# evgueni-ovtchinnikov/raleigh

Hardware: AMD Instinct MI355X
Metric: inner-iter GB/s vs HBM roofline (Gram+dots+SpMM of one block-JCG iteration) (higher is better)
Workload: dtype f64; 1 GPU; block-JCG inner iteration: 9 Gram + 4 dots + 1 SpMM, n=215x215x215=9938375 rows (9938375 per GPU), m=32, 7-pt Laplacian nnz=69291275, rows sharded over 1 GPU(s), strong scaling; n=9938375, m=32, nnz=69291275

## Files before the change

### raleigh_amd/csrc/gram.hip

```cpp
#include <stdlib.h>

#include "common.h"

namespace rlh {

template <typename R> struct Mfma16;
template <> struct Mfma16<double> {
  typedef double acc_t __attribute__((ext_vector_type(4)));
  static __device__ __forceinline__ acc_t run(double a, double b, acc_t c) {
    return __builtin_amdgcn_mfma_f64_16x16x4f64(a, b, c, 0, 0, 0);
  }
  static __device__ __forceinline__ int out_row(int lane, int reg) { return (lane >> 4) + 4 * reg; }
};
template <> struct Mfma16<float> {
  typedef float acc_t __attribute__((ext_vector_type(4)));
  static __device__ __forceinline__ acc_t run(float a, float b, acc_t c) {
    return __builtin_amdgcn_mfma_f32_16x16x4f32(a, b, c, 0, 0, 0);
  }
  static __device__ __forceinline__ int out_row(int lane, int reg) { return (lane >> 4) * 4 + reg; }
};

struct GramSeg { const void *p; int64_t ld; int c0; };
constexpr int kGramSegs = 4;

// ... 889 lines not shown
    a.npj = (vx + 127) / 128;
    a.nchunks = (n + 256 / (int)sizeof(R) - 1) / (256 / (int)sizeof(R));
    if (a.same && vx <= 128)
      return gram_launch<DT, 4, 2, true, 0, false, true, true>(a, 1, 1, my, mx, d_out);
    return gram_launch<DT, 4, 2, true, 0, false, true>(a, (vy + 127) / 128, a.npj, my, mx, d_out);
  }
  if (aligned && vx > 32 && vy > 32 && vx <= 64 && vy <= 64 && env_quad()) {
    a.npj = 1;
    a.nchunks = (n + 512 / (int)sizeof(R) - 1) / (512 / (int)sizeof(R));
    if (a.same) return gram_launch<DT, 2, 1, true, 0, false, true, true>(a, 1, 1, my, mx, d_out);
    return gram_launch<DT, 2, 1, true, 0, false, true>(a, 1, 1, my, mx, d_out);
  }
  const int ROWS = (mode == 3 ? 2 : (mode == 4 ? 4 : 1)) * 512 / (int)sizeof(R);
  a.nchunks = (n + ROWS - 1) / ROWS;
#define RLH_GRAM_CASE(pi, pj)                                                              \
  if (PI == pi && PJ == pj) {                                                              \
    if constexpr (pi * pj <= 4)        \
      if (mode == 1) return gram_launch<DT, pi, pj, true, 1>(a, npi, npj, my, mx, d_out);  \
    if constexpr (pi <= 2 && pj <= 2)         \
      if (mode == 3) return gram_launch<DT, pi, pj, true, 3>(a, npi, npj, my, mx, d_out);  \
    if constexpr (pi * pj == 1)                                                            \
      if (mode == 4) return gram_launch<DT, pi, pj, true, 4>(a, npi, npj, my, mx, d_out);  \
    if constexpr (pi == pj && pi <= 2)                                                     \
      if (mode == 2) return gram_launch<DT, pi, pj, true, 2>(a, npi, npj, my, mx, d_out);  \
    return aligned ? gram_launch<DT, pi, pj, true, 0>(a, npi, npj, my, mx, d_out)          \
                   : gram_launch<DT, pi, pj, false, 0>(a, npi, npj, my, mx, d_out);        \
  }
  RLH_GRAM_CASE(1, 1) RLH_GRAM_CASE(1, 2) RLH_GRAM_CASE(1, 4)
  RLH_GRAM_CASE(2, 1) RLH_GRAM_CASE(2, 2) RLH_GRAM_CASE(2, 4)
  RLH_GRAM_CASE(4, 1) RLH_GRAM_CASE(4, 2) RLH_GRAM_CASE(4, 4)
#undef RLH_GRAM_CASE
  set_error("rlh_gram: no kernel for panel %d x %d", PI, PJ);
  return 1;
}

template <int DT>
static int gram_multi_impl(int64_t n, int nx, const void *const *X, const int64_t *ldx, const int64_t *mx, int ny,
                           const void *const *Y, const int64_t *ldy, const int64_t *my, void *d_out) {
  using R = typename DType<DT>::R;
  constexpr int NC = DType<DT>::cplx ? 2 : 1;
  Context &c = ctx();
  GramArgs a;
  const int64_t es = dtype_size(DT);
  bool aligned = true;
  int64_t mxt = 0, myt = 0;
  for (int k = 0; k < nx; ++k) {
    a.xs[k] = GramSeg{X[k], ldx[k], (int)mxt};
    mxt += mx[k];
    aligned = aligned && aligned16(X[k], ldx[k], es);
  }
  for (int k = 0; k < ny; ++k) {
    a.ys[k] = GramSeg{Y[k], ldy[k], (int)myt};
    myt += my[k];
    aligned = aligned && aligned16(Y[k], ldy[k], es);
  }
  for (int k = nx; k < kGramSegs; ++k) a.xs[k] = GramSeg{nullptr, 0, 1 << 30};
  for (int k = ny; k < kGramSegs; ++k) a.ys[k] = GramSeg{nullptr, 0, 1 << 30};
  a.nxs = nx; a.nys = ny;
  const int vx = (int)mxt * NC, vy = (int)myt * NC;
  const int PI = pick_tiles(vy), PJ = pick_tiles(vx);
  const int npi = (vy + PI * 16 - 1) / (PI * 16), npj = (vx + PJ * 16 - 1) / (PJ * 16);
  a.X = X[0]; a.Y = Y[0]; a.ldx = ldx[0]; a.ldy = ldy[0]; a.n = n; a.mx = (int)mxt; a.my = (int)myt;
  a.same = 0; a.npj = npj; a.partials = c.work;
  a.nt = gram_nt(n * (mxt + myt) * es);
  {
    const int stream = getenv("RLH_GRAM_STREAM") ? atoi(getenv("RLH_GRAM_STREAM")) : 1;
    if (stream && aligned && vx <= 64 && vy <= 64 && (vx > 8 || vy > 8)) {
      a.npj = 1;
      a.xal = -1;
      if (!DType<DT>::cplx && nx == 1 && mxt > 16 && mxt <= 32 && myt > 32)
        for (int k2 = 0; k2 < ny; ++k2)
          if (Y[k2] == X[0] && ldy[k2] == ldx[0] && my[k2] == mx[0] && a.ys[k2].c0 % 16 == 0) a.xal = a.ys[k2].c0;
      return gram_stream_launch<DT>(a, myt, mxt, d_out);
    }
  }
  if (nx == 1 && npi * npj > 1) {
    for (int k = 0; k < ny; ++k)
      if (int rc = gram_impl<DT>(n, mx[0], X[0], ldx[0], my[k], Y[k], ldy[k],
                                 (char *)d_out + (size_t)a.ys[k].c0 * (size_t)mxt * (size_t)es))
        return rc;
    return 0;
  }
  const int ROWS = 512 / (int)sizeof(R);
  a.nchunks = (n + ROWS - 1) / ROWS;
#define RLH_GRAM_MCASE(pi, pj)                                                                        \
  if (PI == pi && PJ == pj)                                                                           \
    return aligned ? gram_launch<DT, pi, pj, true, 0, true>(a, npi, npj, myt, mxt, d_out)             \
                   : gram_launch<DT, pi, pj, false, 0, true>(a, npi, npj, myt, mxt, d_out);
  RLH_GRAM_MCASE(1, 1) RLH_GRAM_MCASE(1, 2) RLH_GRAM_MCASE(1, 4)
  RLH_GRAM_MCASE(2, 1) RLH_GRAM_MCASE(2, 2) RLH_GRAM_MCASE(2, 4)
  RLH_GRAM_MCASE(4, 1) RLH_GRAM_MCASE(4, 2) RLH_GRAM_MCASE(4, 4)
#undef RLH_GRAM_MCASE
  set_error("rlh_gram_multi: no kernel for panel %d x %d", PI, PJ);
  return 1;
}

template <typename T, bool ALIGNED, bool NT>
__global__ __launch_bounds__(256) void dots_kernel(const T *X, int64_t ldx, const T *Y, int64_t ldy, int64_t n,
                                                   T *partials, int nbx, int per) {
  constexpr int VEC = 16 / (int)sizeof(T);
  const int col = blockIdx.y;
  const T *x = X + (int64_t)col * ldx;
  const T *y = Y + (int64_t)col * ldy;
  T acc = zero_of(T{});
  struct alignas(16) V { T v[VEC]; };
  typedef unsigned u4 __attribute__((ext_vector_type(4)));
  auto piece = [&](const T *p) -> V {
    union { u4 u; V v; } c;
    if constexpr (NT) c.u = __builtin_nontemporal_load(reinterpret_cast<const u4 *>(p));
    else c.u = *reinterpret_cast<const u4 *>(p);
    return c.v;
  };
  for (int g = 0; g < per; g += 4) {
    const int64_t base = ((int64_t)blockIdx.x * per + g) * 256 * VEC;
    if (base >= n) break;
    if (ALIGNED && base + 4 * 256 * VEC <= n && x == y) {
      V xv[4];
#pragma unroll
      for (int i = 0; i < 4; ++i) xv[i] = piece(x + base + ((int64_t)i * 256 + threadIdx.x) * VEC);
#pragma unroll
      for (int i = 0; i < 4; ++i)
#pragma unroll
        for (int e = 0; e < VEC; ++e) fma_conj_acc(acc, xv[i].v[e], xv[i].v[e]);
    } else if (ALIGNED && base + 4 * 256 * VEC <= n) {
      V xv[4], yv[4];
#pragma unroll
      for (int i = 0; i < 4; ++i) {
        const int64_t r = base + ((int64_t)i * 256 + threadIdx.x) * VEC;
        xv[i] = piece(x + r);
        yv[i] = piece(y + r);
      }
#pragma unroll
      for (int i = 0; i < 4; ++i)
#pragma unroll
        for (int e = 0; e < VEC; ++e) fma_conj_acc(acc, yv[i].v[e], xv[i].v[e]);
    } else {
      for (int i = 0; i < 4; ++i) {
        const int64_t r = base + ((int64_t)i * 256 + threadIdx.x) * VEC;
        for (int e = 0; e < VEC && r + e < n; ++e) fma_conj_acc(acc, y[r + e], x[r + e]);
      }
    }
  }
  __shared__ T red[256];
  red[threadIdx.x] = acc;
  __syncthreads();
  for (int s = 128; s > 0; s >>= 1) {
    if (threadIdx.x < s) red[threadIdx.x] = add_of(red[threadIdx.x], red[threadIdx.x + s]);
    __syncthreads();
  }
  if (threadIdx.x == 0) partials[(int64_t)col * nbx + blockIdx.x] = red[0];
}

template <typename T>
__global__ __launch_bounds__(256) void dots_finalize(const T *partials, int nbx, int m, T *out) {
  const int lane = threadIdx.x & 63;
  const int col = blockIdx.x * 4 + (threadIdx.x >> 6);
  if (col >= m) return;
  T s = zero_of(T{});
  for (int b = lane; b < nbx; b += 64) s = add_of(s, partials[(int64_t)col * nbx + b]);
  if constexpr (sizeof(T) == sizeof(float) || sizeof(T) == sizeof(double)) {
    using R = T;
#pragma unroll
    for (int off = 32; off > 0; off >>= 1) s = s + (R)__shfl_xor(s, off);
  }
  if (lane == 0) out[col] = s;
}

template <typename R2, typename C>
__device__ __forceinline__ C shfl_complex(C v, int off) {
  C r;
  r.re = __shfl_xor(v.re, off);
  r.im = __shfl_xor(v.im, off);
  return r;
}

template <>
__global__ __launch_bounds__(256) void dots_finalize<c32>(const c32 *partials, int nbx, int m, c32 *out) {
  const int lane = threadIdx.x & 63;
  const int col = blockIdx.x * 4 + (threadIdx.x >> 6);
  if (col >= m) return;
  c32 s = zero_of(c32{});
  for (int b = lane; b < nbx; b += 64) s = add_of(s, partials[(int64_t)col * nbx + b]);
#pragma unroll
  for (int off = 32; off > 0; off >>= 1) s = add_of(s, shfl_complex<float>(s, off));
  if (lane == 0) out[col] = s;
}

template <>
__global__ __launch_bounds__(256) void dots_finalize<c64>(const c64 *partials, int nbx, int m, c64 *out) {
  const int lane = threadIdx.x & 63;
  const int col = blockIdx.x * 4 + (threadIdx.x >> 6);
  if (col >= m) return;
  c64 s = zero_of(c64{});
  for (int b = lane; b < nbx; b += 64) s = add_of(s, partials[(int64_t)col * nbx + b]);
#pragma unroll
  for (int off = 32; off > 0; off >>= 1) s = add_of(s, shfl_complex<double>(s, off));
  if (lane == 0) out[col] = s;
}

template <int DT>
static int dots_impl(int64_t n, int64_t m, const void *X, int64_t ldx, const void *Y, int64_t ldy, void *d_out) {
  using T = typename DType<DT>::T;
  Context &c = ctx();
  constexpr int VEC = 16 / (int)sizeof(T);
  int per = 4;
  int64_t nbx = (n + 256 * VEC * (int64_t)per - 1) / (256 * VEC * (int64_t)per);
  while (nbx > 2048 || (nbx > 1 && (size_t)nbx * m * sizeof(T) > kWorkspaceBytes / 4)) {
    per += 4;
    nbx = (n + 256 * VEC * (int64_t)per - 1) / (256 * VEC * (int64_t)per);
  }
  if (nbx < 1) nbx = 1;
  RLH_REQUIRE((size_t)nbx * m * sizeof(T) <= kWorkspaceBytes, "rlh_dots: too many columns");
  const int nt = gram_nt(n * m * (int64_t)sizeof(T) * (X == Y ? 1 : 2));
  const bool aligned = aligned16(X, ldx, sizeof(T)) && aligned16(Y, ldy, sizeof(T));
  dim3 grid((unsigned)nbx, (unsigned)m);
  if (aligned && (nt & 1))
    hipLaunchKernelGGL((dots_kernel<T, true, true>), grid, dim3(256), 0, c.stream, (const T *)X, ldx, (const T *)Y, ldy,
                       n, (T *)c.work, (int)nbx, per);
  else if (aligned)
    hipLaunchKernelGGL((dots_kernel<T, true, false>), grid, dim3(256), 0, c.stream, (const T *)X, ldx, (const T *)Y, ldy,
                       n, (T *)c.work, (int)nbx, per);
  else
    hipLaunchKernelGGL((dots_kernel<T, false, false>), grid, dim3(256), 0, c.stream, (const T *)X, ldx, (const T *)Y, ldy,
                       n, (T *)c.work, (int)nbx, per);
  RLH_HIP(hipGetLastError());
  hipLaunchKernelGGL((dots_finalize<T>), dim3(((int)m + 3) / 4), dim3(256), 0, c.stream, (const T *)c.work,
                     (int)nbx, (int)m, (T *)d_out);
  RLH_HIP(hipGetLastError());
  return 0;
}

template <typename R>
__global__ __launch_bounds__(256) void absmax_kernel(const R *X, int64_t ldx_r, int64_t n_r, double *partials, int nbx) {
  const R *x = X + (int64_t)blockIdx.y * ldx_r;
  double mx = 0.0;
  const int64_t stride = (int64_t)gridDim.x * 256;
  for (int64_t r = (int64_t)blockIdx.x * 256 + threadIdx.x; r < n_r; r += stride) {
    const double v = fabs((double)x[r]);
    mx = v > mx ? v : mx;
  }
  __shared__ double red[256];
  red[threadIdx.x] = mx;
  __syncthreads();
  for (int s = 128; s > 0; s >>= 1) {
    if (threadIdx.x < s) red[threadIdx.x] = red[threadIdx.x] > red[threadIdx.x + s] ? red[threadIdx.x] : red[threadIdx.x + s];
    __syncthreads();
  }
  if (threadIdx.x == 0) partials[(int64_t)blockIdx.y * nbx + blockIdx.x] = red[0];
}

__global__ __launch_bounds__(256) void absmax_finalize(const double *partials, int64_t count, double *out) {
  double mx = 0.0;
  for (int64_t i = threadIdx.x; i < count; i += 256) mx = partials[i] > mx ? partials[i] : mx;
  __shared__ double red[256];
  red[threadIdx.x] = mx;
  __syncthreads();
  for (int s = 128; s > 0; s >>= 1) {
    if (threadIdx.x < s) red[threadIdx.x] = red[threadIdx.x] > red[threadIdx.x + s] ? red[threadIdx.x] : red[threadIdx.x + s];
    __syncthreads();
  }
  if (threadIdx.x == 0) out[0] = red[0];
}

template <int DT>
static int absmax_impl(int64_t n, int64_t m, const void *X, int64_t ldx, void *d_out) {
  using R = typename DType<DT>::R;
  constexpr int NC = DType<DT>::cplx ? 2 : 1;
  Context &c = ctx();
  int64_t nbx = (n * NC + 256 * 8 - 1) / (256 * 8);
  const int64_t cap = ((int64_t)c.num_cu * 8 + m - 1) / m;
  if (nbx > cap) nbx = cap;
  if (nbx < 1) nbx = 1;
  RLH_REQUIRE((size_t)nbx * m * sizeof(double) <= kWorkspaceBytes, "rlh_absmax: too many columns");
  hipLaunchKernelGGL((absmax_kernel<R>), dim3((unsigned)nbx, (unsigned)m), dim3(256), 0, c.stream, (const R *)X,
                     ldx * NC, n * NC, (double *)c.work, (int)nbx);
  RLH_HIP(hipGetLastError());
  hipLaunchKernelGGL(absmax_finalize, dim3(1), dim3(256), 0, c.stream, (const double *)c.work, nbx * m, (double *)d_out);
  RLH_HIP(hipGetLastError());
  return 0;
}

template <typename T>
__global__ __launch_bounds__(256) void dots_transp_kernel(const T *X, int64_t ldx, const T *Y, int64_t ldy,
                                                          int64_t n, int m, T *out) {
  const int64_t stride = (int64_t)gridDim.x * blockDim.x;
  for (int64_t r = (int64_t)blockIdx.x * blockDim.x + threadIdx.x; r < n; r += stride) {
    T acc = zero_of(T{});
    for (int i = 0; i < m; ++i) fma_conj_acc(acc, Y[r + (int64_t)i * ldy], X[r + (int64_t)i * ldx]);
    out[r] = acc;
  }
}

template <int DT>
static int dots_transp_impl(int64_t n, int64_t m, const void *X, int64_t ldx, const void *Y, int64_t ldy,
                            void *d_out) {
  using T = typename DType<DT>::T;
  Context &c = ctx();
  int64_t nb = (n + 255) / 256;
  if (nb > (int64_t)c.num_cu * 8) nb = (int64_t)c.num_cu * 8;
  hipLaunchKernelGGL((dots_transp_kernel<T>), dim3((unsigned)nb), dim3(256), 0, c.stream, (const T *)X, ldx,
                     (const T *)Y, ldy, n, (int)m, (T *)d_out);
  RLH_HIP(hipGetLastError());
  return 0;
}

}

using namespace rlh;

#define RLH_DISPATCH(dt, fn, ...)                              \
  switch (dt) {                                                \
    case RLH_S: rc = fn<RLH_S>(__VA_ARGS__); break;            \
    case RLH_D: rc = fn<RLH_D>(__VA_ARGS__); break;            \
    case RLH_C: rc = fn<RLH_C>(__VA_ARGS__); break;            \
    case RLH_Z: rc = fn<RLH_Z>(__VA_ARGS__); break;            \
    default: rlh::set_error("unknown dtype %d", dt); rc = 1;   \
  }

extern "C" {

int rlh_gram(int dtype, int64_t n, int64_t mx, const void *X, int64_t ldx, int64_t my, const void *Y, int64_t ldy,
             void *d_out, void *h_out) {
  if (int rc = require_ready()) return rc;
  RLH_REQUIRE(dtype_valid(dtype), "rlh_gram: unknown dtype %d", dtype);
  RLH_REQUIRE(n >= 0 && mx >= 0 && my >= 0, "rlh_gram: negative size");
  RLH_REQUIRE(mx <= 32768 && my <= 32768, "rlh_gram: more than 32768 vectors in a window");
  if (mx == 0 || my == 0) return 0;
  RLH_REQUIRE(X && Y, "rlh_gram: null block pointer");
  RLH_REQUIRE(ldx >= n && ldy >= n, "rlh_gram: leading dimension smaller than n");
  RLH_REQUIRE(d_out || h_out, "rlh_gram: no output buffer");
  const size_t bytes = (size_t)(mx * my * dtype_size(dtype));
  if (!d_out) {
    if (int rc = ensure_result(bytes)) return rc;
    d_out = ctx().result_hd;
  }
  int rc = 0;
  if (n == 0) {
    RLH_HIP(hipMemsetAsync(d_out, 0, bytes, ctx().stream));
  } else {
    RLH_DISPATCH(dtype, gram_impl, n, mx, X, ldx, my, Y, ldy, d_out)
  }
  if (rc) return rc;
  if (h_out) return fetch_result(h_out, d_out, bytes);
  return 0;
}

int rlh_gram_multi(int dtype, int64_t n, int nx, const void *const *X, const int64_t *ldx, const int64_t *mx, int ny,
// ... 89 lines not shown
```

### raleigh_amd/csrc/spmm.hip

```cpp
#include <unordered_map>

#include "spmm.h"

namespace rlh {

template <typename T, int JT, int TT, bool CHEB>
__global__ __launch_bounds__(256, (JT * TT >= 64 ? 1 : 2)) void sell_spmm_kernel(const int64_t *__restrict__ slice_ptr,
                                                        const int32_t *__restrict__ cols,
                                                        const T *__restrict__ vals, int64_t n_rows,
                                                        int64_t n_slices, const T *__restrict__ X, int64_t ldx,
                                                        int64_t n_own, const T *__restrict__ H, int64_t ldh,
                                                        T *__restrict__ Y, int64_t ldy, int m, int chunk,
                                                        int ntiles, int tiles_per_block, ChebArgs<T> cheb) {
  const int lane = threadIdx.x & 63;
  const int wave = threadIdx.x >> 6;
  const int xcd = blockIdx.x & 7;
  const int slices_per_block = 4 / tiles_per_block;
  const int64_t q0 = (int64_t)(blockIdx.x >> 3) * slices_per_block + wave / tiles_per_block;
  const int64_t q_stride = (int64_t)(gridDim.x >> 3) * slices_per_block;
  const int64_t nchunks = (n_slices + chunk - 1) / chunk;
  for (int tile = wave % tiles_per_block; tile < ntiles; tile += tiles_per_block) {
    const int j0 = tile * JT;
    const int jv = (m - j0) < JT ? (m - j0) : JT;
    const T *__restrict__ Xp = X + (int64_t)j0 * ldx;
// ... 443 lines not shown
      scol[i] = gsrc[mt.goff + g + lane / LPG] + (lane % LPG) * EPL;
    }
    auto stage_load = [&](int s, VecU<T, EPL> (&st)[SLOTS]) {
#pragma unroll
      for (int i = 0; i < SLOTS; ++i) {
        int j = s * cps + scc[i];
        if (j > m - 1) j = m - 1;
        st[i] = *reinterpret_cast<const VecU<T, EPL> *>(X + (int64_t)j * ldx + scol[i]);
      }
    };
    auto stage_write = [&](int s, const VecU<T, EPL> (&st)[SLOTS]) {
      unsigned boff = (unsigned)(s & 1) * (unsigned)kStkBufBytes;
      asm volatile("" : "+s"(boff));
#pragma unroll
      for (int i = 0; i < SLOTS; ++i) {
        VecA<T, EPL> val;
#pragma unroll
        for (int k = 0; k < EPL; ++k) val.e[k] = st[i].e[k];
        *reinterpret_cast<VecA<T, EPL> *>(ldsb + (lane16 + (boff + (unsigned)sbase[i]))) = val;
      }
    };
    auto compute = [&](int s) {
      unsigned boff = (unsigned)(s & 1) * (unsigned)kStkBufBytes;
      int j = s * cps;
      const int jend = (j + cps < m) ? j + cps : m;
      for (; j < jend; ++j) {
        asm volatile("" : "+s"(boff));
#pragma unroll
        for (int r = 0; r < R; ++r) {
          T acc = zero_of(T{});
#pragma unroll
          for (int t = 0; t < WMAX; ++t) {
            if constexpr (!PACK) {
              fma_acc(acc, v[r][t], *reinterpret_cast<const T *>(ldsb + (ixb[r][t] + boff)));
            } else if ((t & 1) == 0) {
              unsigned w = ixb[r][t / 2];
              asm volatile("" : "+v"(w));
              fma_acc(acc, v[r][t], *reinterpret_cast<const T *>(ldsb + ((w & 0xffffu) * (unsigned)sizeof(T) + boff)));
              fma_acc(acc, v[r][t + 1], *reinterpret_cast<const T *>(ldsb + ((w >> 16) * (unsigned)sizeof(T) + boff)));
            }
          }
          if (row[r] < n_rows) nt_store(Y + row[r] + (int64_t)j * ldy, acc);
        }
        boff += (unsigned)F * (unsigned)sizeof(T);
      }
    };
    if constexpr (sizeof(T) >= 8) {
      VecU<T, EPL> stA[SLOTS];
      stage_load(0, stA);
      stage_write(0, stA);
      __syncthreads();
      for (int s = 0; s + 1 < nsteps; ++s) {
        stage_load(s + 1, stA);
        compute(s);
        stage_write(s + 1, stA);
        __syncthreads();
      }
      compute(nsteps - 1);
      __syncthreads();
      continue;
    }
    VecU<T, EPL> stA[SLOTS], stB[SLOTS];
    stage_load(0, stA);
    stage_load(nsteps > 1 ? 1 : 0, stB);
    stage_write(0, stA);
    __syncthreads();
    int s = 0;
    for (; s + 3 < nsteps; s += 2) {
      stage_load(s + 2, stA);
      compute(s);
      stage_write(s + 1, stB);
      __syncthreads();
      stage_load(s + 3, stB);
      compute(s + 1);
      stage_write(s + 2, stA);
      __syncthreads();
    }
    const int left = nsteps - s;
    if (left == 3) {
      stage_load(s + 2, stA);
      compute(s);
      stage_write(s + 1, stB);
      __syncthreads();
      compute(s + 1);
      stage_write(s + 2, stA);
      __syncthreads();
      compute(s + 2);
    } else if (left == 2) {
      compute(s);
      stage_write(s + 1, stB);
      __syncthreads();
      compute(s + 1);
    } else {
      compute(s);
    }
    __syncthreads();
  }
}

template <int N> __device__ __forceinline__ void wait_vm_le() { asm volatile("s_waitcnt vmcnt(%0)" :: "n"(N) : "memory"); }

__device__ __forceinline__ void wait_vm_outstanding(int n) {
#define RLH_WC(k) case k: wait_vm_le<k>(); break;
#define RLH_WC8(k) RLH_WC(k) RLH_WC(k + 1) RLH_WC(k + 2) RLH_WC(k + 3) RLH_WC(k + 4) RLH_WC(k + 5) RLH_WC(k + 6) RLH_WC(k + 7)
  switch (n) {
    RLH_WC8(0) RLH_WC8(8) RLH_WC8(16)
    default: wait_vm_le<0>(); break;
  }
#undef RLH_WC8
#undef RLH_WC
}

constexpr int kStkLdsBytes = 160 * 1024;
template <typename T> struct StkRing { static constexpr int NB = sizeof(T) >= 16 ? 2 : 4, SLOT = kStkLdsBytes / NB; };

__device__ __forceinline__ void stk_touch(float &v) { asm volatile("" : "+v"(v)); }
__device__ __forceinline__ void stk_touch(double &v) { asm volatile("" : "+v"(v)); }
__device__ __forceinline__ void stk_touch(c32 &v) { asm volatile("" : "+v"(v.re), "+v"(v.im)); }
__device__ __forceinline__ void stk_touch(c64 &v) { asm volatile("" : "+v"(v.re), "+v"(v.im)); }

__device__ __forceinline__ void stk_store(float *p, float v) { __builtin_nontemporal_store(v, p); }
__device__ __forceinline__ void stk_store(double *p, double v) { __builtin_nontemporal_store(v, p); }
__device__ __forceinline__ void stk_store(c32 *p, c32 v) {
  typedef float f32x2 __attribute__((ext_vector_type(2)));
  __builtin_nontemporal_store(f32x2{v.re, v.im}, reinterpret_cast<f32x2 *>(p));
}
__device__ __forceinline__ void stk_store(c64 *p, c64 v) {
  typedef double f64x2 __attribute__((ext_vector_type(2)));
  __builtin_nontemporal_store(f64x2{v.re, v.im}, reinterpret_cast<f64x2 *>(p));
}

template <typename T, int R, int LD, int DBG = 0, bool CHEB = false>
__global__ __launch_bounds__(1024) void well_stack_dma_kernel(const WellMeta *__restrict__ meta,
                                                              const int32_t *__restrict__ member,
                                                              const int32_t *__restrict__ gsrc,
                                                              const uint16_t *__restrict__ idx,
                                                              const T *__restrict__ vals, const int32_t *__restrict__ pat,
                                                              const uint16_t *__restrict__ dtab, int64_t n_rows,
                                                              const int32_t *__restrict__ sched, int64_t sched_len,
                                                              const T *__restrict__ X, int64_t ldx, int64_t n_own,
                                                              const T *__restrict__ H, int64_t ldh,
                                                              T *__restrict__ Y, int64_t ldy, int m, ChebArgs<T> cheb) {
  constexpr int WMAX = 8;
  constexpr int NB = StkRing<T>::NB, D = NB - 1;
  static_assert(!CHEB || NB == 2, "the fused step drains the ring every vector: two slots only");
  constexpr int SLOT = StkRing<T>::SLOT;
  constexpr int EPL = 16 / (int)sizeof(T);
  constexpr int LPG = 64 / EPL;
  static_assert((D - 1) * LD + D * R < 24, "wait_vm_outstanding's cases");
  extern __shared__ __align__(16) char ldsb[];
  const int tid = threadIdx.x;
  const int lane = tid & 63;
  const int wave = __builtin_amdgcn_readfirstlane(tid >> 6);
  for (int64_t pos = blockIdx.x; pos < sched_len; pos += gridDim.x) {
    const int64_t sb = sched[pos];
    if (sb < 0) continue;
    const WellMeta mt = meta[sb];
    const int ng = mt.width_ng >> 8;
    int row[R];
    T v[R][WMAX];
    unsigned ixb[R][WMAX / 2];
    bool whole = true;
    int nmem = 0;
#pragma unroll
    for (int r = 0; r < R; ++r) {
      const int2 mr = reinterpret_cast<const int2 *>(member)[sb * R + r];
      if (mr.y > 0) {
        nmem = r + 1;
        whole = whole && mr.y == kWellRows;
      }
      row[r] = tid < mr.y ? mr.x + tid : -1;
      unsigned px[WMAX];
      if (sizeof(T) < 16 && pat) well_load_entries_pat<T, WMAX>(vals, pat, dtab, idx, mt.eoff + 8 * r, sb * R + r, tid, v[r], px);
      else well_load_entries<T, WMAX>(vals, idx, mt.eoff + 8 * r, tid, WMAX, v[r], px);
#pragma unroll
      for (int t = 0; t < WMAX; t += 2) ixb[r][t / 2] = px[t] | (px[t + 1] << 16);
    }
    int scol[LD];
    const int npieces = ng / EPL;
    const int nw = __builtin_amdgcn_readfirstlane((npieces + LD - 1) / LD);
    const int mine = __builtin_amdgcn_readfirstlane(wave < nw ? (npieces - wave + nw - 1) / nw : 0);
#pragma unroll
    for (int i = 0; i < LD; ++i) {
      int q = (wave + nw * i) * EPL;
      if (q > ng - EPL) q = ng - EPL;
      scol[i] = gsrc[mt.goff + q + lane / LPG] + (lane % LPG) * EPL;
    }
#pragma unroll
    for (int r = 0; r < R; ++r) {
#pragma unroll
      for (int t = 0; t < WMAX; ++t) stk_touch(v[r][t]);
#pragma unroll
      for (int t = 0; t < WMAX / 2; ++t) asm volatile("" : "+v"(ixb[r][t]));
    }
#pragma unroll
    for (int i = 0; i < LD; ++i) asm volatile("" : "+v"(scol[i]));
    auto issue = [&](int j) {
      const unsigned slot = (unsigned)(j & (NB - 1)) * (unsigned)SLOT;
      const T *src = X + (int64_t)j * ldx;
      const T *hsrc = H ? H + (int64_t)j * ldh - n_own : src;
#pragma unroll
      for (int i = 0; i < LD; ++i) {
        if (i >= mine || (DBG & 1)) break;
        const T *g = (scol[i] < n_own ? src : hsrc) + scol[i];
        unsigned dst = slot + (unsigned)(wave + nw * i) * 1024u, keep;
        asm volatile("s_mov_b32 %0, m0\n\ts_mov_b32 m0, %2\n\ts_nop 0\n\tglobal_load_lds_dwordx4 %1, off\n\ts_mov_b32 m0, %0"
                     : "=&s"(keep) : "v"(g), "s"(dst) : "memory");
      }
    };
    auto compute = [&](int j) {
      unsigned boff = (unsigned)(j & (NB - 1)) * (unsigned)SLOT;
      asm volatile("" : "+s"(boff));
#pragma unroll
      for (int r = 0; r < R; ++r) {
        if (r >= nmem) break;
        T acc = zero_of(T{});
#pragma unroll
        for (int t = 0; t < WMAX; t += 2) {
          unsigned w = ixb[r][t / 2];
          asm volatile("" : "+v"(w));
          if constexpr ((DBG & 2) != 0) acc = (t == (j & 6)) ? v[r][t] : acc;
          else {
            fma_acc(acc, v[r][t], *reinterpret_cast<const T *>(ldsb + ((w & 0xffffu) * (unsigned)sizeof(T) + boff)));
            fma_acc(acc, v[r][t + 1], *reinterpret_cast<const T *>(ldsb + ((w >> 16) * (unsigned)sizeof(T) + boff)));
          }
        }
        if constexpr ((DBG & 4) != 0) { if (ixb[r][0] == 0xfffffffeu) Y[(int64_t)row[r] + (int64_t)j * ldy] = acc; }
        else if constexpr ((DBG & 8) != 0) { if (whole || row[r] >= 0) Y[(int64_t)row[r] + (int64_t)j * ldy] = acc; }
        else if (whole || row[r] >= 0) stk_store(Y + (int64_t)row[r] + (int64_t)j * ldy, acc);
      }
    };
    __builtin_amdgcn_s_barrier();
    if constexpr (CHEB) {
      issue(0);
      for (int j = 0; j < m; ++j) {
        if (j == 0) wait_vm_outstanding(0);
        __builtin_amdgcn_s_barrier();
        if (j + 1 < m) issue(j + 1);
        unsigned boff = (unsigned)(j & (NB - 1)) * (unsigned)SLOT;
        asm volatile("" : "+s"(boff));
#pragma unroll
        for (int r = 0; r < R; ++r) {
          if (r >= nmem) break;
          T acc = zero_of(T{});
#pragma unroll
          for (int t = 0; t < WMAX - 2; t += 2) {
            unsigned w = ixb[r][t / 2];
            asm volatile("" : "+v"(w));
            fma_acc(acc, v[r][t], *reinterpret_cast<const T *>(ldsb + ((w & 0xffffu) * (unsigned)sizeof(T) + boff)));
            fma_acc(acc, v[r][t + 1], *reinterpret_cast<const T *>(ldsb + ((w >> 16) * (unsigned)sizeof(T) + boff)));
          }
          unsigned w = ixb[r][WMAX / 2 - 1];
          asm volatile("" : "+v"(w));
          fma_acc(acc, v[r][WMAX - 2], *reinterpret_cast<const T *>(ldsb + ((w & 0xffffu) * (unsigned)sizeof(T) + boff)));
          const T yv = *reinterpret_cast<const T *>(ldsb + ((w >> 16) * (unsigned)sizeof(T) + boff));
          T out = sub_of(scale_of(cheb.cy, yv), scale_of(cheb.cb, acc));
          const bool live = whole || row[r] >= 0;
          T *pp = Y + (int64_t)row[r] + (int64_t)j * ldy;
          T pv = zero_of(T{}), bv = zero_of(T{});
          if (live) {
            pv = *pp;
            bv = cheb.B[(int64_t)row[r] + (int64_t)j * cheb.ldb];
          }
          wait_vm_outstanding(0);
          stk_touch(pv);
          stk_touch(bv);
          out = add_of(add_of(out, scale_of(cheb.cp, pv)), scale_of(cheb.cb, bv));
          if (live) stk_store(pp, out);
        }
      }
      continue;
    }
    for (int j = 0; j < D && j < m; ++j) issue(j);
    for (int j = 0; j < m; ++j) {
      const int later = m - 1 - j < D - 1 ? m - 1 - j : D - 1;
      wait_vm_outstanding(((DBG & 1) ? 0 : later * mine) + ((DBG & 16) && whole ? (j < D ? j : D) * nmem : 0));
      __builtin_amdgcn_s_barrier();
      if (j + D < m) issue(j + D);
      compute(j);
    }
  }
}

__device__ __forceinline__ float bf16_to_f32(unsigned short h) { return __uint_as_float((unsigned)h << 16); }
__device__ __forceinline__ unsigned short f32_to_bf16(float f) {
  unsigned u = __float_as_uint(f);
  u += 0x7FFFu + ((u >> 16) & 1u);
  return (unsigned short)(u >> 16);
}
__device__ __forceinline__ float cheb_update(float cy, float y, float cp, float p, float cb, float b, float t) {
  return __fmaf_rn(cy, y, __fmaf_rn(cp, p, __fmul_rn(cb, __fsub_rn(b, t))));
}
struct alignas(16) Bf8 { unsigned short e[8]; };
struct alignas(8) Bf8U { unsigned short e[8]; };

constexpr int kBfCps = 8;
constexpr int kBfBufBytes = 56 * 1024;

template <int WMAX>
__global__ __launch_bounds__(1024) void well_cheb_bf16_kernel(const WellMeta *__restrict__ meta,
                                                              const int32_t *__restrict__ gsrc,
                                                              const uint16_t *__restrict__ idx,
                                                              const float *__restrict__ vals, int64_t n_rows,
                                                              const int32_t *__restrict__ sched, int64_t sched_len,
                                                              const unsigned short *__restrict__ Yk, int64_t ldy,
                                                              int64_t n_own, const unsigned short *__restrict__ H,
                                                              int64_t ldh,
                                                              unsigned short *__restrict__ P, int64_t ldp,
                                                              const unsigned short *__restrict__ B, int64_t ldb,
                                                              int m, float cy, float cp, float cb) {
  constexpr int SLOTS = 4;
  __shared__ __attribute__((aligned(16))) char ldsb[2 * kBfBufBytes + 16 * kBfCps * 64 * 4];
  const int tid = threadIdx.x;
  const int lane = tid & 63;
  const int wave = __builtin_amdgcn_readfirstlane(tid >> 6);
  float *tile = reinterpret_cast<float *>(ldsb + 2 * kBfBufBytes) + wave * (kBfCps * 64);
  for (int64_t pos = blockIdx.x; pos < sched_len; pos += gridDim.x) {
    const int64_t b = sched[pos];
    if (b < 0) continue;
    const WellMeta mt = meta[b];
    const int width = mt.width_ng & 255;
    const int ng = mt.width_ng >> 8;
    const int F2 = ng * 128;
    int cps = kBfBufBytes / F2;
    if (cps > kBfCps) cps = kBfCps;
    if (cps > m) cps = m;
    const int nsteps = (m + cps - 1) / cps;
    const int G = ng * cps;
    const int64_t row0 = b * kWellRows + (int64_t)wave * 64;
    const int64_t row = row0 + lane;
    float v[WMAX];
    unsigned ixb[WMAX];
    well_load_entries<float, WMAX>(vals, idx, mt.eoff, tid, width, v, ixb);
#pragma unroll
    for (int t = 0; t < WMAX; ++t) ixb[t] *= 2u;
    int sbase[SLOTS], scc[SLOTS], scol[SLOTS];
#pragma unroll
    for (int i = 0; i < SLOTS; ++i) {
      int q = (wave + 16 * i) * 8;
      if (q > G - 8) q = G - 8;
      const int cc = q / ng, g = q - cc * ng;
      scc[i] = __builtin_amdgcn_readfirstlane(cc);
      sbase[i] = __builtin_amdgcn_readfirstlane(cc * F2 + g * 128);
      scol[i] = gsrc[mt.goff + g + lane / 8] + (lane % 8) * 8;
    }
    Bf8U stA[SLOTS], stB[SLOTS];
    auto stage_load = [&](int s, Bf8U (&st)[SLOTS]) {
#pragma unroll
      for (int i = 0; i < SLOTS; ++i) {
        int j = s * cps + scc[i];
        if (j > m - 1) j = m - 1;
        const int c = scol[i];
        const unsigned short *src = c < n_own ? Yk + (int64_t)j * ldy + c : H + (int64_t)j * ldh + (c - n_own);
        st[i] = *reinterpret_cast<const Bf8U *>(src);
      }
    };
    auto stage_write = [&](int s, const Bf8U (&st)[SLOTS]) {
      unsigned boff = (unsigned)(s & 1) * (unsigned)kBfBufBytes;
      asm volatile("" : "+s"(boff));
#pragma unroll
      for (int i = 0; i < SLOTS; ++i) {
        Bf8 val;
#pragma unroll
        for (int k = 0; k < 8; ++k) val.e[k] = st[i].e[k];
        *reinterpret_cast<Bf8 *>(ldsb + ((unsigned)lane * 16u + (boff + (unsigned)sbase[i]))) = val;
      }
    };
    auto compute = [&](int s) {
      unsigned boff = (unsigned)(s & 1) * (unsigned)kBfBufBytes;
      const int j0 = s * cps;
      const int c8 = lane >> 3, rg = lane & 7;
      const int j = j0 + c8;
      const int64_t r8 = row0 + rg * 8;
      const bool mine = c8 < cps && j < m && r8 < n_rows;
      const bool whole = mine && r8 + 8 <= n_rows;
      const int jc = j < m ? j : m - 1;
      const int64_t rc = whole ? r8 : 0;
      unsigned short *pp = P + (int64_t)jc * ldp + rc;
      const Bf8 pv = *reinterpret_cast<const Bf8 *>(pp);
      const Bf8 bv = *reinterpret_cast<const Bf8 *>(B + (int64_t)jc * ldb + rc);
      const Bf8 yv = *reinterpret_cast<const Bf8 *>(Yk + (int64_t)jc * ldy + rc);
#pragma unroll 1
      for (int c = 0; c < cps; ++c) {
        unsigned bo = boff + (unsigned)c * (unsigned)F2;
        asm volatile("" : "+s"(bo));
        float acc = 0.f;
        if (j0 + c < m) {
#pragma unroll
          for (int t = 0; t < WMAX; ++t)
            acc = fmaf(v[t], bf16_to_f32(*reinterpret_cast<const unsigned short *>(ldsb + (ixb[t] + bo))), acc);
        }
        tile[c * 64 + lane] = acc;
      }
      const int ct = c8 < cps ? c8 : 0;
      float t8[8];
      {
        const float4 lo = *reinterpret_cast<const float4 *>(tile + ct * 64 + rg * 8);
        const float4 hi = *reinterpret_cast<const float4 *>(tile + ct * 64 + rg * 8 + 4);
        t8[0] = lo.x; t8[1] = lo.y; t8[2] = lo.z; t8[3] = lo.w;
        t8[4] = hi.x; t8[5] = hi.y; t8[6] = hi.z; t8[7] = hi.w;
      }
      if (whole) {
        Bf8 out;
#pragma unroll
        for (int k = 0; k < 8; ++k)
          out.e[k] = f32_to_bf16(cheb_update(cy, bf16_to_f32(yv.e[k]), cp, bf16_to_f32(pv.e[k]), cb, bf16_to_f32(bv.e[k]), t8[k]));
        *reinterpret_cast<Bf8 *>(pp) = out;
      } else if (mine) {
        unsigned short *pq = P + (int64_t)j * ldp + r8;
        const unsigned short *bq = B + (int64_t)j * ldb + r8, *yq = Yk + (int64_t)j * ldy + r8;
        for (int k = 0; k < 8 && r8 + k < n_rows; ++k)
          pq[k] = f32_to_bf16(cheb_update(cy, bf16_to_f32(yq[k]), cp, bf16_to_f32(pq[k]), cb, bf16_to_f32(bq[k]), t8[k]));
      }
    };
    stage_load(0, stA);
    stage_load(1, stB);
    stage_write(0, stA);
    __syncthreads();
    int s = 0;
    for (; s + 3 < nsteps; s += 2) {
      stage_load(s + 2, stA);
      compute(s);
      stage_write(s + 1, stB);
      __syncthreads();
      stage_load(s + 3, stB);
      compute(s + 1);
      stage_write(s + 2, stA);
      __syncthreads();
    }
// ... 141 lines not shown
      const int jv = j0 + c8;
      const int jc = jv < m ? jv : m - 1;
#pragma unroll
      for (int r = 0; r < R; ++r) {
        if (r >= nmem) break;
        const int64_t r8 = row0[r] + rg * 8;
        const int64_t rc = r8 + 8 <= n_rows ? r8 : 0;
        if constexpr ((DBG & 4) != 0) continue;
        dma16(P + (int64_t)jc * ldp + rc, opbase + (unsigned)(r * 3 + 0) * 1024u);
        dma16(B + (int64_t)jc * ldb + rc, opbase + (unsigned)(r * 3 + 1) * 1024u);
        dma16(Yk + (int64_t)jc * ldy + rc, opbase + (unsigned)(r * 3 + 2) * 1024u);
      }
    };
    operands(0);
    for (int j0 = 0; j0 < m; j0 += 8) {
      const int cnt = m - j0 < 8 ? m - j0 : 8;
      const int jv = j0 + c8;
      const bool act = c8 < cnt;
      float acc[R][8];
#pragma unroll
      for (int jj = 0; jj < 8; jj += VPS) {
#pragma unroll
        for (int u = 0; u < VPS; ++u)
#pragma unroll
          for (int r = 0; r < R; ++r) acc[r][jj + u] = 0.f;
        if (jj < cnt) {
          const int j = j0 + jj;
          if (!whole) wait_vm_le<0>();
          else if (mine) wait_vm_outstanding(jj == 0 && !(DBG & 4) ? 3 * nmem : 0);
          __builtin_amdgcn_s_barrier();
          const int jn = jj + VPS < cnt ? j + VPS : j0 + 8;
          if (jn < m) issue(jn, par ^ 1u);
          unsigned boff = par * (unsigned)SLOT;
          asm volatile("" : "+s"(boff));
#pragma unroll
          for (int u = 0; u < VPS; ++u) {
#pragma unroll
            for (int r = 0; r < R; ++r) {
              if (r >= nmem) break;
              float a = 0.f;
              if constexpr ((DBG & 2) != 0) a = v[r][(jj + u) & 7];
              else
#pragma unroll
              for (int t = 0; t < WMAX; t += 2) {
                unsigned w = ixb[r][t / 2];
                asm volatile("" : "+v"(w));
                a = fmaf(v[r][t], bf16_to_f32(*reinterpret_cast<const unsigned short *>(ldsb + ((w & 0xffffu) * 2u + boff))), a);
                a = fmaf(v[r][t + 1], bf16_to_f32(*reinterpret_cast<const unsigned short *>(ldsb + ((w >> 16) * 2u + boff))), a);
              }
              acc[r][jj + u] = a;
            }
            boff += (unsigned)IMG;
          }
          par ^= 1u;
        }
      }
      if (cnt <= VPS || !mine || !whole) wait_vm_le<0>();
      rlh_u32x4e outs[R];
#pragma unroll
      for (int r = 0; r < R; ++r) {
        if (r >= nmem) break;
        if constexpr ((DBG & 4) != 0) { if (acc[r][0] == 1.2345e30f) P[0] = 0; continue; }
        union { rlh_u32x4e u; unsigned short e[8]; } pu, bu, yu, ou;
        pu.u = *reinterpret_cast<const rlh_u32x4e *>(ldsb + opbase + (unsigned)(r * 3 + 0) * 1024u + (unsigned)lane * 16u);
        bu.u = *reinterpret_cast<const rlh_u32x4e *>(ldsb + opbase + (unsigned)(r * 3 + 1) * 1024u + (unsigned)lane * 16u);
        yu.u = *reinterpret_cast<const rlh_u32x4e *>(ldsb + opbase + (unsigned)(r * 3 + 2) * 1024u + (unsigned)lane * 16u);
        asm volatile("s_waitcnt lgkmcnt(0)" ::: "memory");
        float *tile = reinterpret_cast<float *>(ldsb + opbase + (unsigned)(r * 3) * 1024u);
#pragma unroll
        for (int jj = 0; jj < 8; ++jj) tile[jj * 64 + lane] = acc[r][jj];
        float t8[8];
        {
          const float4 lo = *reinterpret_cast<const float4 *>(tile + c8 * 64 + rg * 8);
          const float4 hi = *reinterpret_cast<const float4 *>(tile + c8 * 64 + rg * 8 + 4);
          t8[0] = lo.x; t8[1] = lo.y; t8[2] = lo.z; t8[3] = lo.w;
          t8[4] = hi.x; t8[5] = hi.y; t8[6] = hi.z; t8[7] = hi.w;
        }
        const int64_t r8 = row0[r] + rg * 8;
        if (whole || r8 + 8 <= n_rows) {
#pragma unroll
          for (int k = 0; k < 8; ++k)
            ou.e[k] = f32_to_bf16(cheb_update(cy, bf16_to_f32(yu.e[k]), cp, bf16_to_f32(pu.e[k]), cb, bf16_to_f32(bu.e[k]), t8[k]));
          outs[r] = ou.u;
        } else if (act && r8 < n_rows) {
          unsigned short *pq = P + (int64_t)jv * ldp + r8;
          const unsigned short *bq = B + (int64_t)jv * ldb + r8, *yq = Yk + (int64_t)jv * ldy + r8;
          for (int k = 0; k < 8 && r8 + k < n_rows; ++k)
            pq[k] = f32_to_bf16(cheb_update(cy, bf16_to_f32(yq[k]), cp, bf16_to_f32(pq[k]), cb, bf16_to_f32(bq[k]), t8[k]));
        }
      }
      asm volatile("s_waitcnt lgkmcnt(0)" ::: "memory");
      if (j0 + 8 < m) operands(j0 + 8);
      if constexpr ((DBG & 4) == 0) {
#pragma unroll
        for (int r = 0; r < R; ++r) {
          if (r >= nmem) break;
          const int64_t r8 = row0[r] + rg * 8;
          if ((whole || r8 + 8 <= n_rows) && act) *reinterpret_cast<rlh_u32x4e *>(P + (int64_t)jv * ldp + r8) = outs[r];
        }
      }
    }
  }
}

template <typename T>
static int launch_stack(const rlh_csr *h, int part, int64_t m, const T *X, int64_t ldx, int64_t n_own, const T *H,
                        int64_t ldh, T *Y, int64_t ldy, bool dma, const ChebArgs<T> *cheb = nullptr) {
  Context &c = ctx();
  const int32_t *sched = part == 0 ? h->stk_sched : h->stk_sched_part[part - 1];
  const int64_t sched_len = part == 0 ? h->stk_sched_len : h->stk_sched_part_len[part - 1];
  const int grid = part == 0 ? h->stk_grid : h->stk_grid_part[part - 1];
  if (grid == 0) return 0;
  constexpr bool cplx = std::is_same<T, c32>::value || std::is_same<T, c64>::value;
  if (dma) {
    constexpr int EPL = 16 / (int)sizeof(T);
    const int32_t *pat = sizeof(T) < 16 && env_int("RLH_SPMM_STACK_PAT", 1) != 0 ? h->stk_pat : nullptr;
    const int ld = 5;
#define RLH_STK_DMA(LD_, ...)                                                                                           \
    do {                                                                                                                \
      static bool attr_dma = false;                                                                                     \
      if (!attr_dma) {                                                                                                  \
        RLH_HIP(hipFuncSetAttribute(reinterpret_cast<const void *>(&well_stack_dma_kernel<T, kStkR, LD_ __VA_ARGS__>),  \
                                    hipFuncAttributeMaxDynamicSharedMemorySize, kStkLdsBytes));                         \
        attr_dma = true;                                                                                                \
      }                                                                                                                 \
      hipLaunchKernelGGL((well_stack_dma_kernel<T, kStkR, LD_ __VA_ARGS__>), dim3((unsigned)grid), dim3(1024),          \
                         kStkLdsBytes, c.stream, h->stk_meta, h->stk_member, h->stk_gsrc, h->stk_idx,                   \
                         pat ? (const T *)h->stk_table : (const T *)h->stk_vals, pat, pat ? h->stk_dtab : nullptr,      \
                         h->n_rows, sched, sched_len, X, ldx, n_own, H, ldh, Y, ldy, (int)m,                            \
                         cheb ? *cheb : ChebArgs<T>{});                                                                 \
    } while (0)
    const int dbg = env_int("RLH_SPMM_STACK_DBG", 0);
    RLH_REQUIRE(h->stk_gmax <= 80 * EPL, "rlh_spmm: a stack of %d staging groups", h->stk_gmax);
    if (cheb) {
      if constexpr (sizeof(T) == 16) {
        RLH_STK_DMA(5, , 0, true);
        RLH_HIP(hipGetLastError());
        return 0;
      } else {
        RLH_REQUIRE(false, "rlh_spmm_cheb: the stacked fused step exists for 16-byte elements only");
      }
    }
    if (dbg && std::is_same<T, double>::value) {
      if constexpr (std::is_same<T, double>::value) {
        switch (dbg) {
          case 1: RLH_STK_DMA(5, , 1); break;
          case 2: RLH_STK_DMA(5, , 2); break;
          case 3: RLH_STK_DMA(5, , 3); break;
          case 4: RLH_STK_DMA(5, , 4); break;
          case 5: RLH_STK_DMA(5, , 5); break;
          case 6: RLH_STK_DMA(5, , 6); break;
          case 7: RLH_STK_DMA(5, , 7); break;
          case 8: RLH_STK_DMA(5, , 8); break;
          default: RLH_STK_DMA(5, , 16); break;
        }
      }
    } else RLH_STK_DMA(5);
#undef RLH_STK_DMA
    RLH_HIP(hipGetLastError());
    return 0;
  }
  RLH_REQUIRE(part == 0 && H == nullptr, "rlh_spmm: the register-staged stack kernel takes the whole operator only");
  if constexpr (!cplx) {
    static bool attr = false;
    if (!attr) {
      RLH_HIP(hipFuncSetAttribute(reinterpret_cast<const void *>(&well_stack_kernel<T, kStkR>),
                                  hipFuncAttributeMaxDynamicSharedMemorySize, 2 * kStkBufBytes));
      attr = true;
    }
    const int cps_cap = env_int("RLH_SPMM_CPS", 8);
    hipLaunchKernelGGL((well_stack_kernel<T, kStkR>), dim3((unsigned)h->stk_grid), dim3(1024), 2 * kStkBufBytes, c.stream,
                       h->stk_meta, h->stk_member, h->stk_gsrc, h->stk_idx, (const T *)h->stk_vals, h->n_rows, h->stk_sched,
                       h->stk_sched_len, X, ldx, Y, ldy, (int)m, cps_cap < 1 ? 1 : cps_cap);
    RLH_HIP(hipGetLastError());
  }
  return 0;
}

template <typename T>
static int launch_well(const rlh_csr *h, int part, int64_t m, const T *X, int64_t ldx, int64_t n_own, const T *H,
                       int64_t ldh, T *Y, int64_t ldy, const ChebArgs<T> *cheb) {
  return launch_well_w<T, 8>(h, part, m, X, ldx, n_own, H, ldh, Y, ldy, cheb);
}

static int well_split(rlh_csr *h, int64_t n_own);
static int stack_split(rlh_csr *h, int64_t n_own);

template <typename T>
static int stack_dispatch(rlh_csr *h, int part, int64_t m, const T *X, int64_t ldx, int64_t n_own, const T *H, int64_t ldh,
                          T *Y, int64_t ldy, bool *done, const ChebArgs<T> *cheb = nullptr) {
  constexpr bool cplx = std::is_same<T, c32>::value || std::is_same<T, c64>::value;
  constexpr int EPL = 16 / (int)sizeof(T);
  *done = false;
  if (h->stk_blocks == 0 || env_int("RLH_SPMM_STACK", 1) == 0) return 0;
  bool dma = h->stk_gmax * 64 * (int)sizeof(T) <= StkRing<T>::SLOT && (cplx || env_int("RLH_SPMM_STACK_DMA", 1) != 0);
  if (cplx && !dma) return 0;
  if (sizeof(T) == 4 && !cplx && part == 0 && H == nullptr && env_int("RLH_SPMM_STACK_DMA", 1) < 2) dma = false;
  if (h->stk_overhang > 0 && (H != nullptr && n_own != h->n_cols ? ldh < h->n_cols - n_own + h->stk_overhang
                                                                  : ldx < h->n_cols + h->stk_overhang)) {
    static bool said = false;
    if (!said && env_int("RLH_SPMM_VERBOSE", 0) != 0) {
      said = true;
      fprintf(stderr, "rlh_spmm_part: stacks not used (overhang %d, ldh %lld, ldx %lld, n_cols %lld, n_own %lld)\n", h->stk_overhang,
              (long long)ldh, (long long)ldx, (long long)h->n_cols, (long long)n_own);
    }
    return 0;
  }
  if (part != 0 || H != nullptr) {
    if (!dma || (H != nullptr && n_own != h->n_cols && !(h->stk_aligned && n_own % EPL == 0))) {
      static bool said = false;
      if (!said && env_int("RLH_SPMM_VERBOSE", 0) != 0) {
        said = true;
        fprintf(stderr, "rlh_spmm_part: stacks not used (dma %d, aligned %d, n_own %lld, gmax %d, overhang %d)\n", (int)dma,
                h->stk_aligned, (long long)n_own, h->stk_gmax, h->stk_overhang);
      }
      return 0;
    }
    if (part != 0)
      if (int rc = stack_split(h, n_own)) return rc;
  }
  if (cheb && !dma) return 0;
  *done = true;
  return launch_stack<T>(h, part, m, X, ldx, n_own, H, ldh, Y, ldy, dma, cheb);
}

template <int DT>
static int spmm_impl(rlh_csr *h, int part, int64_t m, const void *X_, int64_t ldx, int64_t n_own, const void *H_,
                     int64_t ldh, void *Y_, int64_t ldy, const void *B_ = nullptr, int64_t ldb = 0, double cy = 0.0,
                     double cp = 0.0, double cb = 0.0) {
  using T = typename DType<DT>::T;
  constexpr int JTMAX = DType<DT>::cplx ? 16 : 32;
  const T *X = (const T *)X_, *H = (const T *)H_;
  T *Y = (T *)Y_;
  ChebArgs<T> cargs{(const T *)B_, ldb, cy, cp, cb};
  const ChebArgs<T> *cheb = B_ ? &cargs : nullptr;
  if (cheb == nullptr && (DType<DT>::cplx || h->well_blocks > 0)) {
    bool done = false;
    const int rc = stack_dispatch<T>(h, part, m, X, ldx, n_own, H, ldh, Y, ldy, &done);
    if (rc || done) return rc;
  }
  if (cheb != nullptr && sizeof(T) == 16 && env_int("RLH_SPMM_STACK_CHEB", 1) != 0) {
    bool done = false;
    if (h->stk_self) {
      const int rc = stack_dispatch<T>(h, part, m, X, ldx, n_own, H, ldh, Y, ldy, &done, cheb);
      if (rc || done) return rc;
    }
    {
      static bool said = false;
      if (!said && env_int("RLH_SPMM_VERBOSE", 0) != 0) {
        said = true;
        fprintf(stderr, "rlh_spmm_cheb: stacked fused step not used (stacks %lld, self %d, part %d, halo %d, n_own %lld, n_cols %lld, gmax %d, aligned %d)\n",
                (long long)h->stk_blocks, h->stk_self, part, H != nullptr, (long long)n_own, (long long)h->n_cols, h->stk_gmax, h->stk_aligned);
      }
    }
    RLH_REQUIRE(env_int("RLH_SPMM_STACK_CHEB", 1) < 2, "rlh_spmm_cheb: the stacked fused step does not take this operator or call");
  }
  if (h->wide_blocks > 0) {
    switch (DT) {
      case RLH_S: return wide_spmm_s(h, part, m, X_, ldx, n_own, H_, ldh, Y_, ldy, B_, ldb, cy, cp, cb);
      case RLH_D: return wide_spmm_d(h, part, m, X_, ldx, n_own, H_, ldh, Y_, ldy, B_, ldb, cy, cp, cb);
      case RLH_C: return wide_spmm_c(h, part, m, X_, ldx, n_own, H_, ldh, Y_, ldy, B_, ldb, cy, cp, cb);
      default:    return wide_spmm_z(h, part, m, X_, ldx, n_own, H_, ldh, Y_, ldy, B_, ldb, cy, cp, cb);
    }
  }
  if constexpr (!DType<DT>::cplx) {
    if (h->well_blocks > 0) {
      if (part != 0)
        if (int rc = well_split(h, n_own)) return rc;
      return launch_well<T>(h, part, m, X, ldx, n_own, H, ldh, Y, ldy, cheb);
    }
  }
  if (part == 1) return 0;
  const int jt_cap = env_int("RLH_SPMM_JT", 16);
  if (m <= 4 || jt_cap <= 4) return launch_spmm<T, 4>(h, m, X, ldx, n_own, H, ldh, Y, ldy, cheb);
  if (m <= 8 || jt_cap <= 8) return launch_spmm<T, 8>(h, m, X, ldx, n_own, H, ldh, Y, ldy, cheb);
  if (m <= 16 || JTMAX == 16 || jt_cap <= 16 || cheb) return launch_spmm<T, 16>(h, m, X, ldx, n_own, H, ldh, Y, ldy, cheb);
  return launch_spmm<T, (JTMAX == 32 ? 32 : 16)>(h, m, X, ldx, n_own, H, ldh, Y, ldy, cheb);
}

template <typename T>
__global__ __launch_bounds__(256) void gather_rows_kernel(const int64_t *__restrict__ idx, int64_t nidx,
                                                          const T *__restrict__ X, int64_t ldx,
                                                          T *__restrict__ Out, int64_t ldo) {
  const T *x = X + (int64_t)blockIdx.y * ldx;
  T *o = Out + (int64_t)blockIdx.y * ldo;
  const int64_t stride = (int64_t)gridDim.x * 256;
  for (int64_t i = (int64_t)blockIdx.x * 256 + threadIdx.x; i < nidx; i += stride) o[i] = x[idx[i]];
}

template <int DT>
static int gather_rows_impl(int64_t nidx, const int64_t *d_idx, int64_t m, const void *X, int64_t ldx, void *Out,
                            int64_t ldo) {
  using T = typename DType<DT>::T;
  Context &c = ctx();
  int64_t nb = (nidx + 255) / 256;
  const int64_t cap = ((int64_t)c.num_cu * 8 + m - 1) / m;
  if (nb > cap) nb = cap;
  if (nb < 1) nb = 1;
  hipLaunchKernelGGL((gather_rows_kernel<T>), dim3((unsigned)nb, (unsigned)m), dim3(256), 0, c.stream, d_idx, nidx,
                     (const T *)X, ldx, (T *)Out, ldo);
  RLH_HIP(hipGetLastError());
  return 0;
}

template <int DT>
static int csr_build(rlh_csr *h, const int64_t *indptr, const int32_t *indices, const void *values_) {
// ... 984 lines not shown
```

Baseline: 6476 GB/s.

## Pair adjacent-row SpMM outputs into 16-byte stores; batch dots finalize loads

In the stacked SpMM kernel, when a well holds two full row groups with even start and Y is 16-byte aligned, each lane pair swaps results through a DPP quad permute. Each lane then writes a 16-byte f64x2 with a nontemporal store, halving the number of store instructions. The vmcnt wait is skipped when a wave issued no DMA loads, and new debug variants are wired in. The dots finalize reduction now loads partials in unrolled runs of 32 (16 for 16-byte types) so more loads are in flight. The trade-offs are more register pressure and an alignment-dependent path.

```diff
diff --git a/raleigh_amd/csrc/gram.hip b/raleigh_amd/csrc/gram.hip
--- a/raleigh_amd/csrc/gram.hip
+++ b/raleigh_amd/csrc/gram.hip
@@ -1065,12 +1065,26 @@
 }
 
 template <typename T>
+__device__ __forceinline__ T dots_lane_sum(const T *p, int lane, int nbx) {
+  constexpr int RUN = sizeof(T) >= 16 ? 16 : 32;
+  T s = zero_of(T{});
+  for (int b0 = lane; b0 < nbx; b0 += 64 * RUN) {
+    T x[RUN];
+#pragma unroll
+    for (int i = 0; i < RUN; ++i) x[i] = b0 + 64 * i < nbx ? p[b0 + 64 * i] : zero_of(T{});
+#pragma unroll
+    for (int i = 0; i < RUN; ++i)
+      if (b0 + 64 * i < nbx) s = add_of(s, x[i]);
+  }
+  return s;
+}
+
+template <typename T>
 __global__ __launch_bounds__(256) void dots_finalize(const T *partials, int nbx, int m, T *out) {
   const int lane = threadIdx.x & 63;
   const int col = blockIdx.x * 4 + (threadIdx.x >> 6);
   if (col >= m) return;
-  T s = zero_of(T{});
-  for (int b = lane; b < nbx; b += 64) s = add_of(s, partials[(int64_t)col * nbx + b]);
+  T s = dots_lane_sum(partials + (int64_t)col * nbx, lane, nbx);
   if constexpr (sizeof(T) == sizeof(float) || sizeof(T) == sizeof(double)) {
     using R = T;
 #pragma unroll
@@ -1092,8 +1106,7 @@
   const int lane = threadIdx.x & 63;
   const int col = blockIdx.x * 4 + (threadIdx.x >> 6);
   if (col >= m) return;
-  c32 s = zero_of(c32{});
-  for (int b = lane; b < nbx; b += 64) s = add_of(s, partials[(int64_t)col * nbx + b]);
+  c32 s = dots_lane_sum(partials + (int64_t)col * nbx, lane, nbx);
 #pragma unroll
   for (int off = 32; off > 0; off >>= 1) s = add_of(s, shfl_complex<float>(s, off));
   if (lane == 0) out[col] = s;
@@ -1104,8 +1117,7 @@
   const int lane = threadIdx.x & 63;
   const int col = blockIdx.x * 4 + (threadIdx.x >> 6);
   if (col >= m) return;
-  c64 s = zero_of(c64{});
-  for (int b = lane; b < nbx; b += 64) s = add_of(s, partials[(int64_t)col * nbx + b]);
+  c64 s = dots_lane_sum(partials + (int64_t)col * nbx, lane, nbx);
 #pragma unroll
   for (int off = 32; off > 0; off >>= 1) s = add_of(s, shfl_complex<double>(s, off));
   if (lane == 0) out[col] = s;
diff --git a/raleigh_amd/csrc/spmm.hip b/raleigh_amd/csrc/spmm.hip
--- a/raleigh_amd/csrc/spmm.hip
+++ b/raleigh_amd/csrc/spmm.hip
@@ -619,6 +619,8 @@
   const int tid = threadIdx.x;
   const int lane = tid & 63;
   const int wave = __builtin_amdgcn_readfirstlane(tid >> 6);
+  constexpr bool PAIRABLE = std::is_same<T, double>::value && R == 2 && !CHEB && (DBG & 32) == 0;
+  const bool y16 = ((uintptr_t)Y & 15) == 0 && (ldy & 1) == 0;
   for (int64_t pos = blockIdx.x; pos < sched_len; pos += gridDim.x) {
     const int64_t sb = sched[pos];
     if (sb < 0) continue;
@@ -629,12 +631,14 @@
     unsigned ixb[R][WMAX / 2];
     bool whole = true;
     int nmem = 0;
+    int odd_first = 0;
 #pragma unroll
     for (int r = 0; r < R; ++r) {
       const int2 mr = reinterpret_cast<const int2 *>(member)[sb * R + r];
       if (mr.y > 0) {
         nmem = r + 1;
         whole = whole && mr.y == kWellRows;
+        odd_first |= mr.x;
       }
       row[r] = tid < mr.y ? mr.x + tid : -1;
       unsigned px[WMAX];
@@ -675,23 +679,43 @@
                      : "=&s"(keep) : "v"(g), "s"(dst) : "memory");
       }
     };
+    auto product = [&](int r, int j, unsigned boff) -> T {
+      T acc = zero_of(T{});
+#pragma unroll
+      for (int t = 0; t < WMAX; t += 2) {
+        unsigned w = ixb[r][t / 2];
+        asm volatile("" : "+v"(w));
+        if constexpr ((DBG & 2) != 0) acc = (t == (j & 6)) ? v[r][t] : acc;
+        else {
+          fma_acc(acc, v[r][t], *reinterpret_cast<const T *>(ldsb + ((w & 0xffffu) * (unsigned)sizeof(T) + boff)));
+          fma_acc(acc, v[r][t + 1], *reinterpret_cast<const T *>(ldsb + ((w >> 16) * (unsigned)sizeof(T) + boff)));
+        }
+      }
+      return acc;
+    };
+    bool pair = false;
+    if constexpr (PAIRABLE) pair = whole && nmem == 2 && (odd_first & 1) == 0 && y16;
     auto compute = [&](int j) {
       unsigned boff = (unsigned)(j & (NB - 1)) * (unsigned)SLOT;
       asm volatile("" : "+s"(boff));
+      if constexpr (PAIRABLE) {
+        if (pair) {
+          typedef double f64x2 __attribute__((ext_vector_type(2)));
+          const T a0 = product(0, j, boff), a1 = product(1, j, boff);
+          const int q = lane & 1;
+          const T got = dpp_quad<T, 0xB1>(q ? a0 : a1);
+          const f64x2 out = q ? f64x2{got, a1} : f64x2{a0, got};
+          f64x2 *p = reinterpret_cast<f64x2 *>(Y + (int64_t)(q ? row[1] - 1 : row[0]) + (int64_t)j * ldy);
+          if constexpr ((DBG & 4) != 0) { if (ixb[0][0] == 0xfffffffeu) *p = out; }
+          else if constexpr ((DBG & 8) != 0) *p = out;
+          else __builtin_nontemporal_store(out, p);
+          return;
+        }
+      }
 #pragma unroll
       for (int r = 0; r < R; ++r) {
         if (r >= nmem) break;
-        T acc = zero_of(T{});
-#pragma unroll
-        for (int t = 0; t < WMAX; t += 2) {
-          unsigned w = ixb[r][t / 2];
-          asm volatile("" : "+v"(w));
-          if constexpr ((DBG & 2) != 0) acc = (t == (j & 6)) ? v[r][t] : acc;
-          else {
-            fma_acc(acc, v[r][t], *reinterpret_cast<const T *>(ldsb + ((w & 0xffffu) * (unsigned)sizeof(T) + boff)));
-            fma_acc(acc, v[r][t + 1], *reinterpret_cast<const T *>(ldsb + ((w >> 16) * (unsigned)sizeof(T) + boff)));
-          }
-        }
+        const T acc = product(r, j, boff);
         if constexpr ((DBG & 4) != 0) { if (ixb[r][0] == 0xfffffffeu) Y[(int64_t)row[r] + (int64_t)j * ldy] = acc; }
         else if constexpr ((DBG & 8) != 0) { if (whole || row[r] >= 0) Y[(int64_t)row[r] + (int64_t)j * ldy] = acc; }
         else if (whole || row[r] >= 0) stk_store(Y + (int64_t)row[r] + (int64_t)j * ldy, acc);
@@ -741,7 +765,8 @@
     for (int j = 0; j < D && j < m; ++j) issue(j);
     for (int j = 0; j < m; ++j) {
       const int later = m - 1 - j < D - 1 ? m - 1 - j : D - 1;
-      wait_vm_outstanding(((DBG & 1) ? 0 : later * mine) + ((DBG & 16) && whole ? (j < D ? j : D) * nmem : 0));
+      if (mine > 0 || (DBG & 64) != 0)
+        wait_vm_outstanding(((DBG & 1) ? 0 : later * mine) + ((DBG & 16) && whole ? (j < D ? j : D) * (pair ? 1 : nmem) : 0));
       __builtin_amdgcn_s_barrier();
       if (j + D < m) issue(j + D);
       compute(j);
@@ -1189,6 +1214,9 @@
           case 6: RLH_STK_DMA(5, , 6); break;
           case 7: RLH_STK_DMA(5, , 7); break;
           case 8: RLH_STK_DMA(5, , 8); break;
+          case 32: RLH_STK_DMA(5, , 32); break;
+          case 64: RLH_STK_DMA(5, , 64); break;
+          case 96: RLH_STK_DMA(5, , 96); break;
           default: RLH_STK_DMA(5, , 16); break;
         }
       }
```

Result: no change. 6493 GB/s (median of 6 runs) (+0.3%).
